# imedslab/OAProgressionMMF

Hardware: AMD Instinct MI355X
Metric: knees/sec full XR+MRI+clin fusion train step (higher is better)
Workload: dtype f32; 1 GPU; syn3: XR1MR3C1CnnTrf train step (fwd+FocalLoss+bwd+Adam), per-GPU batch 8, global batch 8, BASELINE config 4 on BASELINE's synthetic tensors: XR 1x310x310 + 3 x MRI 1x160x384x384 (slice-major) + 9 clinical; random-init weights; parallelism=dp1, activation_recompute=012,012,01

## Files before the change

oaprogressionmmf_amd/csrc/koaf_bn.hip:

```cpp
#include "koaf_cols.h"

namespace {
template <bool H>
__global__ void __launch_bounds__(256) colstats_kernel(const float* __restrict__ x, int64_t rows, int C,
                                                       ColGeom g, float* __restrict__ part, int sq,
                                                       const float* __restrict__ shift) {
    const int t = threadIdx.x, cvx = t % g.CV, ry = t / g.CV;
    const int c0 = blockIdx.y * g.CW;
    const int64_t rbeg = (int64_t)blockIdx.x * g.rpb;
    const int64_t rend = min(rows, rbeg + (int64_t)g.rpb);
    v4f s[2] = {{0, 0, 0, 0}, {0, 0, 0, 0}};
    v4f k = {0, 0, 0, 0};
    if (shift) k = *(const v4f*)&shift[c0 + 4 * cvx];
    for (int64_t r = rbeg + ry; r < rend; r += g.RP) {
        v4f v = load4<H>(x, r * C + c0 + 4 * cvx) - k;
        s[0] += v;
        s[1] += v * v;
    }
    if (sq) col_block_reduce<2>(s, part, blockIdx.x, C, c0, g.CV, g.RP);
    else {
        v4f s1[1] = {s[0]};
        col_block_reduce<1>(s1, part, blockIdx.x, C, c0, g.CV, g.RP);
    }
}

__global__ void colsum_small_kernel(const float* __restrict__ x, int rows, int C, float* __restrict__ out) {
    int c = blockIdx.x * blockDim.x + threadIdx.x;
    if (c >= C) return;
    float a = 0.f;
    for (int r = 0; r < rows; ++r) a += x[(int64_t)r * C + c];
    out[c] = a;
}
}

extern "C" int koaf_colstats(const float* x, int64_t rows, int32_t C, float* part, int32_t* part_rows,
                             const float* shift, int32_t act16, void* stream) {
    ColGeom g;
    KOAF_REQUIRE(x && part && part_rows && rows > 0, "koaf_colstats: bad args");
    KOAF_REQUIRE(col_geom(rows, C, 1024, &g), "koaf_colstats: unsupported C=%d", C);
    KOAF_LAUNCH_ACT16(act16, colstats_kernel<A16>, dim3(g.nblk, g.nchunk), dim3(256), 0, STREAM, x, rows, C, g, part, 1, shift);
    *part_rows = g.nblk;
    return koaf_check_launch("koaf_colstats");
}
extern "C" int32_t koaf_colpart_rows(int64_t rows, int32_t C) {
    ColGeom g;
    if (!col_geom(rows, C, 1024, &g)) return -1;
    return g.nblk;
}

extern "C" int koaf_colsum(const float* x, float* out, int32_t rows, int32_t C, float* part, void* stream) {
    KOAF_REQUIRE(x && out && rows > 0 && C > 0, "koaf_colsum: bad args");
    ColGeom g;
    if (part && aligned16(x) && col_geom(rows, C, 256, &g)) {
        hipLaunchKernelGGL(colstats_kernel<false>, dim3(g.nblk, g.nchunk), dim3(256), 0, STREAM, x, (int64_t)rows, C, g, part,
                           0, (const float*)nullptr);
        hipLaunchKernelGGL(colfinal_kernel<1>, dim3((C + 63) / 64), dim3(1024), 0, STREAM, part, g.nblk, C, out,
                           (float*)nullptr);
    } else {
        hipLaunchKernelGGL(colsum_small_kernel, dim3((C + 255) / 256), dim3(256), 0, STREAM, x, rows, C, out);
    }
    return koaf_check_launch("koaf_colsum");
}
extern "C" int64_t koaf_colsum_ws(int32_t rows, int32_t C) {
    ColGeom g;
    if (!col_geom(rows, C, 256, &g)) return 0;
    return (int64_t)g.nblk * C;
}

namespace {
__global__ void __launch_bounds__(1024) part_reduce_kernel(const float* __restrict__ src, int rows, int C, int nsum,
                                                           int i1, int chunk, double* __restrict__ ws) {
    __shared__ double red[2][16][64];
    const int cx = threadIdx.x & 63, gy = threadIdx.x >> 6;
    const int c = blockIdx.x * 64 + cx;
    const int r0 = blockIdx.y * chunk, r1 = min(rows, r0 + chunk);
    double a = 0.0, b = 0.0;
    if (c < C)
        for (int r = r0 + gy; r < r1; r += 16) {
            a += (double)src[((int64_t)r * nsum + 0) * C + c];
            b += (double)src[((int64_t)r * nsum + i1) * C + c];
        }
    red[0][gy][cx] = a;
// ... 95 lines not shown
    else
        hipLaunchKernelGGL(bn_finalize_kernel<float>, dim3((C + 63) / 64), dim3(1024), 0, STREAM, stats, rows, C, inv,
                           unbias, gamma, beta, running_mean, running_var, num_batches_tracked, momentum, eps, train,
                           mean, invstd, sc, sh, train ? shift : nullptr, koaf_status_ptr());
    return koaf_check_launch("koaf_bn_finalize");
}

namespace {
template <bool H>
__global__ void __launch_bounds__(256) bn_add_relu_kernel(const float* __restrict__ c, const float* __restrict__ sc,
                                                          const float* __restrict__ sh, const float* __restrict__ idt,
                                                          const float* __restrict__ idsc,
                                                          const float* __restrict__ idsh, float* __restrict__ y,
                                                          int64_t nvec, int C4, uint32_t* status) {
    unsigned nsat = 0;
    for (int64_t i = (int64_t)blockIdx.x * EB + threadIdx.x; i < nvec; i += (int64_t)gridDim.x * EB) {
        const int cv = (int)(i % C4) * 4;
        v4f v = load4_nt<H>(c, i * 4);
        const v4f s4 = *(const v4f*)&sc[cv], h4 = *(const v4f*)&sh[cv];
#pragma unroll
        for (int j = 0; j < 4; ++j) v[j] = fmaf(v[j], s4[j], h4[j]);
        if (idt) {
            v4f d = load4_nt<H>(idt, i * 4);
            if (idsc) {
                const v4f is4 = *(const v4f*)&idsc[cv], ih4 = *(const v4f*)&idsh[cv];
#pragma unroll
                for (int j = 0; j < 4; ++j) d[j] = fmaf(d[j], is4[j], ih4[j]);
            }
            v += d;
        }
#pragma unroll
        for (int j = 0; j < 4; ++j) {
            nsat += !(v[j] * KOAF_ACT_SCALE <= 65504.f) ? 1u : 0u;
            v[j] = v[j] != v[j] ? v[j] : fmaxf(v[j], 0.f);
        }
        store4_nt<H>(y, i * 4, v);
    }
    koaf_status_add(status, 0, nsat);
}
}

extern "C" int koaf_bn_add_relu(const float* c, const float* sc, const float* sh, const float* idt, const float* idsc,
                                const float* idsh, float* y, int64_t rows, int32_t C, int32_t act16, void* stream) {
    KOAF_REQUIRE(c && sc && sh && y && rows > 0 && C > 0 && C % 4 == 0, "koaf_bn_add_relu: bad args");
    KOAF_REQUIRE(aligned16(c) && aligned16(y) && aligned16(sc) && aligned16(sh) && (!idt || aligned16(idt)), "koaf_bn_add_relu: unaligned");
    KOAF_REQUIRE((idsc == nullptr) == (idsh == nullptr), "koaf_bn_add_relu: idsc/idsh come together");
    const int64_t nvec = rows * (C / 4);
    KOAF_LAUNCH_ACT16(act16, bn_add_relu_kernel<A16>, dim3(ew_grid(nvec)), dim3(EB), 0, STREAM, c, sc, sh, idt, idsc, idsh, y,
                      nvec, C / 4, koaf_status_ptr());
    return koaf_check_launch("koaf_bn_add_relu");
}
extern "C" int koaf_bn_relu(const float* c, const float* sc, const float* sh, float* y, int64_t rows, int32_t C,
                            int32_t act16, void* stream) {
    return koaf_bn_add_relu(c, sc, sh, nullptr, nullptr, nullptr, y, rows, C, act16, stream);
}

namespace {
struct PoolGeom { const float* g; const uint8_t* am; int H, W, OH, OW; };
template <bool H, bool POOL>
__global__ void __launch_bounds__(256) bn_bwd_reduce_kernel(const float* __restrict__ g, const float* __restrict__ c,
                                                            const float* __restrict__ ymask,
                                                            const float* __restrict__ sc, const float* __restrict__ sh,
                                                            const float* __restrict__ mean,
                                                            const float* __restrict__ invstd, int mask_mode,
                                                            float* __restrict__ dz_out, int64_t rows, int C,
                                                            ColGeom geo, float* __restrict__ part, float* dz_amax, PoolGeom pg) {
    const int t = threadIdx.x, cvx = t % geo.CV, ry = t / geo.CV;
    unsigned am = 0u;
    const int c0 = blockIdx.y * geo.CW + 4 * cvx;
    const int64_t rbeg = (int64_t)blockIdx.x * geo.rpb;
    const int64_t rend = min(rows, rbeg + (int64_t)geo.rpb);
    const v4f mu = *(const v4f*)&mean[c0], is = *(const v4f*)&invstd[c0];
    v4f s4 = {0, 0, 0, 0}, h4 = {0, 0, 0, 0};
    if (mask_mode == 2) { s4 = *(const v4f*)&sc[c0]; h4 = *(const v4f*)&sh[c0]; }
    v4f s[2] = {{0, 0, 0, 0}, {0, 0, 0, 0}};
    int ix = 0, iy = 0, n = 0;
    if constexpr (POOL) {
        int64_t pp = rbeg + ry;
        ix = (int)(pp % pg.W);
        pp /= pg.W;
        iy = (int)(pp % pg.H);
        n = (int)(pp / pg.H);
    }
    for (int64_t r = rbeg + ry; r < rend; r += geo.RP) {
        const int64_t o = r * C + c0;
        v4f gv;
        if constexpr (POOL) {
            gv = (v4f){0.f, 0.f, 0.f, 0.f};
            const int oya = iy >> 1, oyb = (iy + 1) >> 1, oxa = ix >> 1, oxb = (ix + 1) >> 1;
            const bool vy[2] = {oya < pg.OH, oyb != oya && oyb < pg.OH}, vx[2] = {oxa < pg.OW, oxb != oxa && oxb < pg.OW};
            const int oys[2] = {oya, oyb}, oxs[2] = {oxa, oxb};
            uint32_t a4[4];
            v4f gg[4];
#pragma unroll
            for (int wy = 0; wy < 2; ++wy)
#pragma unroll
                for (int wx = 0; wx < 2; ++wx) {
                    const bool ok = vy[wy] && vx[wx];
                    const int64_t po = ok ? ((int64_t)(n * pg.OH + oys[wy]) * pg.OW + oxs[wx]) * C + c0 : (int64_t)c0;
                    a4[2 * wy + wx] = *(const uint32_t*)&pg.am[po];
                    gg[2 * wy + wx] = *(const v4f*)&pg.g[po];
                }
#pragma unroll
            for (int wy = 0; wy < 2; ++wy)
#pragma unroll
                for (int wx = 0; wx < 2; ++wx) {
                    const bool ok = vy[wy] && vx[wx];
                    const uint32_t want = (uint32_t)((iy - (oys[wy] * 2 - 1)) * 3 + (ix - (oxs[wx] * 2 - 1)));
#pragma unroll
                    for (int j = 0; j < 4; ++j)
                        if (ok && ((a4[2 * wy + wx] >> (8 * j)) & 0xffu) == want) gv[j] += gg[2 * wy + wx][j];
                }
            ix += geo.RP;
            while (ix >= pg.W) { ix -= pg.W; if (++iy == pg.H) { iy = 0; ++n; } }
        } else {
            gv = *(const v4f*)&g[o];
        }
        v4f cvv = load4<H>(c, o);
        if (mask_mode == 1) {
            v4f yv = load4<H>(ymask, o);
#pragma unroll
            for (int j = 0; j < 4; ++j) gv[j] = yv[j] > 0.f ? gv[j] : 0.f;
        } else if (mask_mode == 2) {
#pragma unroll
            for (int j = 0; j < 4; ++j) gv[j] = (cvv[j] * s4[j] + h4[j]) > 0.f ? gv[j] : 0.f;
        }
        if (dz_out) *(v4f*)&dz_out[o] = gv;
        s[0] += gv;
        s[1] += gv * ((cvv - mu) * is);
#pragma unroll
        for (int j = 0; j < 4; ++j) am = max(am, koaf_absbits(gv[j]));
    }
    col_block_reduce<2>(s, part, blockIdx.x, C, blockIdx.y * geo.CW, geo.CV, geo.RP);
    if (dz_amax) block_amax_raise_bits(am, dz_amax);
}
}

extern "C" int koaf_bn_bwd_reduce(const float* g, const float* c, const float* ymask, const float* sc, const float* sh,
                                  const float* mean, const float* invstd, int32_t mask_mode, float* dz_out, float* part,
                                  int32_t* part_rows, int64_t rows, int32_t C, float* dz_amax, int32_t act16, void* stream) {
    ColGeom geo;
    KOAF_REQUIRE(g && c && mean && invstd && part && part_rows && rows > 0, "koaf_bn_bwd_reduce: bad args");
    KOAF_REQUIRE(mask_mode != 1 || ymask, "koaf_bn_bwd_reduce: mask_mode 1 needs ymask");
    KOAF_REQUIRE(mask_mode != 2 || (sc && sh), "koaf_bn_bwd_reduce: mask_mode 2 needs sc/sh");
    KOAF_REQUIRE(col_geom(rows, C, 1024, &geo), "koaf_bn_bwd_reduce: unsupported C=%d", C);
    if (dz_amax && hipMemsetAsync(dz_amax, 0, sizeof(float), STREAM) != hipSuccess) {
        koaf_set_error("koaf_bn_bwd_reduce: memset failed");
        return KOAF_ELAUNCH;
    }
    const PoolGeom nopool{nullptr, nullptr, 0, 0, 0, 0};
    KOAF_LAUNCH_ACT16(act16, (bn_bwd_reduce_kernel<A16, false>), dim3(geo.nblk, geo.nchunk), dim3(256), 0, STREAM, g, c, ymask,
                      sc, sh, mean, invstd, mask_mode, dz_out, rows, C, geo, part, dz_amax, nopool);
    *part_rows = geo.nblk;
    return koaf_check_launch("koaf_bn_bwd_reduce");
}

extern "C" int koaf_bn_bwd_reduce_pool(const float* pool_g, const uint8_t* pool_argmax, const float* c, const float* sc,
                                       const float* sh, const float* mean, const float* invstd, float* dz_out, float* part,
                                       int32_t* part_rows, int32_t N, int32_t H, int32_t W, int32_t C, float* dz_amax,
                                       int32_t act16, void* stream) {
    ColGeom geo;
    KOAF_REQUIRE(pool_g && pool_argmax && c && sc && sh && mean && invstd && dz_out && part && part_rows && N > 0 && H > 0 && W > 0,
                 "koaf_bn_bwd_reduce_pool: bad args");
    const int64_t rows = (int64_t)N * H * W;
    KOAF_REQUIRE(col_geom(rows, C, 1024, &geo), "koaf_bn_bwd_reduce_pool: unsupported C=%d", C);
    if (dz_amax && hipMemsetAsync(dz_amax, 0, sizeof(float), STREAM) != hipSuccess) {
        koaf_set_error("koaf_bn_bwd_reduce_pool: memset failed");
        return KOAF_ELAUNCH;
    }
    const PoolGeom pg{pool_g, pool_argmax, H, W, (H + 2 - 3) / 2 + 1, (W + 2 - 3) / 2 + 1};
    KOAF_LAUNCH_ACT16(act16, (bn_bwd_reduce_kernel<A16, true>), dim3(geo.nblk, geo.nchunk), dim3(256), 0, STREAM, nullptr, c,
                      nullptr, sc, sh, mean, invstd, 2, dz_out, rows, C, geo, part, dz_amax, pg);
    *part_rows = geo.nblk;
    return koaf_check_launch("koaf_bn_bwd_reduce_pool");
}

namespace {
template <typename T>
__global__ void __launch_bounds__(1024) bn_bwd_finalize_kernel(const T* __restrict__ part, int rows, int C,
                                                               double inv_count, const float* __restrict__ sc,
                                                               const float* __restrict__ invstd, float* dgamma,
                                                               float* dbeta, float* coef, int nsum, int i1,
                                                               const float* __restrict__ mean,
                                                               const float* __restrict__ dz_amax, double sqrt_nm1,
                                                               float* amax) {
    __shared__ double red[2][16][64];
    float bound = 0.f;
    const int cx = threadIdx.x & 63, gy = threadIdx.x >> 6;
    const int c = blockIdx.x * 64 + cx;
    double a = 0.0, b = 0.0;
    if (c < C)
        for (int r = gy; r < rows; r += 16) {
            a += (double)part[((int64_t)r * nsum + 0) * C + c];
            b += (double)part[((int64_t)r * nsum + i1) * C + c];
        }
    red[0][gy][cx] = a;
    red[1][gy][cx] = b;
    __syncthreads();
    if (gy == 0 && c < C) {
        double s1 = 0.0, s2 = 0.0;
        for (int j = 0; j < 16; ++j) { s1 += red[0][j][cx]; s2 += red[1][j][cx]; }
        if (dbeta) dbeta[c] = (float)s1;
        if (dgamma) dgamma[c] = (float)s2;
        const float k0 = sc[c], k1 = (float)(s1 * inv_count), k2 = (float)((double)sc[c] * (double)invstd[c] * s2 * inv_count);
        coef[c] = k0;
        coef[C + c] = k1;
        coef[2 * C + c] = k2;
        if (mean) {
            coef[3 * C + c] = k2 * mean[c] - k0 * k1;
            if (amax) bound = fabsf(k0) * ((dz_amax ? *dz_amax : 0.f) + fabsf(k1)) + fabsf(k2) * (float)(sqrt_nm1 / (double)invstd[c]);
        }
    }
    if (amax && mean) block_amax_raise(bound, amax);
}
// ... 243 lines not shown
```

oaprogressionmmf_amd/csrc/koaf_conv.hip:

```cpp
#include "koaf_common.h"

namespace {

inline int64_t rup32(int64_t v) { return (v + 31) / 32 * 32; }

inline void set_fimg(KoafGemm* g, const KoafWImg* w, int R, int64_t K) {
    g->fmt = 1;
    g->A.fscale = KOAF_ACT_SCALE;
    g->B.amax = w->amax;
    if (!w->f) return;
    g->B.kind = 2; g->B.gather = 0;
    g->B.planes = w->f; g->B.ld = rup32(K); g->B.plane_stride = (int64_t)R * g->B.ld;
}

inline void set_aplanes(KoafOperand* a, const uint16_t* planes, int64_t plane_elems) {
    a->kind = 2; a->planes = planes; a->plane_stride = plane_elems; a->zeros = planes + 2 * plane_elems;
    a->ptr = nullptr; a->ptr2 = nullptr; a->tf = 0; a->sc = a->sh = a->sc2 = nullptr;
}

inline void set_gather(KoafOperand* o, int gather, int H, int W, int C, int CS, int PH, int PW, int KH, int KW, int stride, int pad_h,
                       int pad_w) {
    o->gather = gather;
    o->H = H; o->W = W; o->C = C; o->CS = CS;
    o->PH = PH; o->PW = PW;
// ... 188 lines not shown
                g.B.C = Cout; g.B.ld = (int64_t)KH * KW * Cin;
                g.B.KW = g.A.KW; g.B.tap_stride = 2ll * Cin; g.B.tap_stride_h = 2ll * KW * Cin;
                if (ps) {
                    g.B.kind = 2; g.B.gather = 0;
                    g.B.planes = w_dimg + ((int64_t)khs * KW + kws) * Cout; g.B.ld = dld; g.B.plane_stride = dps;
                    g.B.tap_stride = 2ll * Cout; g.B.tap_stride_h = 2ll * KW * Cout;
                }
                if (dy_planes && nkh > 0 && nkw > 0) set_aplanes(&g.A, dy_planes, (int64_t)N * OH * OW * Cout);
                g.M = N * Hc * Wc; g.N = Cin; g.K = nkh * nkw * Cout;
                g.C = dx; g.ldc = Cin;
                g.residual = residual; g.ldr = Cin;
                g.cmap = 1; g.cm_PH = Hc; g.cm_PW = Wc; g.cm_H = H; g.cm_W = W; g.cm_py = py; g.cm_px = px;
                if (bnb) {
                    set_bnb(&g, bnb, part + (int64_t)rows_done * nsum * Cin);
                    rows_done += koaf_gemm_part_rows(&g);
                }
                g.act16 = act16 ? 2 : 0;
                int rc = koaf_gemm(&g, stream);
                if (rc != KOAF_OK) return rc;
            }
        if (part_rows) *part_rows = rows_done;
        return KOAF_OK;
    }
    zero_gemm(&g);
    g.prec = 1;
    if (f16) { g.fmt = 1; g.A.amax = dy_amax; g.B.amax = wimg->amax; }
    g.A.ptr = dy;
    g.A.kind = 0;
    if (dy_apply) set_apply(&g.A, dy_apply, Cout);
    g.B.ptr = w;
    g.B.kind = 1;
    if (is_pointwise(KH, KW, stride, pad)) {
        g.A.gather = 0;
        g.A.ld = Cout;
        g.B.gather = 0;
        g.B.ld = Cin;
    } else {
        set_gather(&g.A, 2, OH, OW, Cout, Cout, H, W, KH, KW, stride, pad, pad);
        g.B.gather = 3;
        g.B.C = Cout;
        g.B.ld = (int64_t)KH * KW * Cin;
        g.B.KW = KW;
        g.B.tap_stride = Cin;
        g.B.tap_stride_h = (int64_t)KW * Cin;
    }
    if (ps) {
        g.B.kind = 2; g.B.gather = 0; g.B.C = 0; g.B.tap_stride = g.B.tap_stride_h = 0;
        g.B.planes = w_dimg; g.B.ld = dld; g.B.plane_stride = dps;
    }
    if (dy_planes) set_aplanes(&g.A, dy_planes, (int64_t)N * OH * OW * Cout);
    g.M = (int)M; g.N = Cin; g.K = KH * KW * Cout;
    g.C = dx; g.ldc = Cin;
    g.residual = residual; g.ldr = Cin;
    if (bnb) {
        set_bnb(&g, bnb, part);
        *part_rows = koaf_gemm_part_rows(&g);
    }
    g.act16 = act16 ? 2 : 0;
    return koaf_gemm(&g, stream);
}

extern "C" int koaf_conv2d_dgrad(const float* dy, const float* w, float* dx, int32_t N, int32_t H, int32_t W,
                                 int32_t Cin, int32_t Cout, int32_t KH, int32_t KW, int32_t stride, int32_t pad,
                                 const float* residual, const KoafWImg* wimg, const float* dy_amax,
                                 const KoafBnApply* dy_apply, const uint16_t* dy_planes, int32_t act16, void* stream) {
    return koaf_conv2d_dgrad_bnb(dy, w, dx, N, H, W, Cin, Cout, KH, KW, stride, pad, residual, nullptr, nullptr,
                                 nullptr, wimg, dy_amax, dy_apply, dy_planes, act16, stream);
}

bool koaf_wgrad3_ring_ok(int N, int H, int W, int Cin, int Cout);
int64_t koaf_wgrad3_ring_ws(int N, int H, int W, int Cin, int Cout);
int koaf_wgrad3_ring(const uint16_t* dy_planes, const uint16_t* x_planes, float* dw, float* slabs, const float* dy_amax,
                     float x_scale, int N, int H, int W, int Cin, int Cout, void* stream);
static inline bool wgrad3_ring_shape(int N, int H, int W, int Cin, int Cout, int KH, int KW, int stride, int pad) {
    return KH == 3 && KW == 3 && stride == 1 && pad == 1 && koaf_wgrad3_ring_ok(N, H, W, Cin, Cout);
}

int koaf_wgrad1(const KoafGemm& g, int bm, int bn, void* stream);
constexpr int WGRAD1_MIN_KCHUNK = 1024;
static inline WgradPlan wgrad1_tile(const KoafGemm& g, const WgradPlan& p) {
    WgradPlan t = {0, 0, p.splitk};
    const KoafOperand& B = g.B;
    if (g.fmt != 1 || g.act16 != 0 || g.A.kind != 1 || B.kind != 1 || g.A.gather || (B.gather != 0 && B.gather != 1)) return t;
    if (g.M % 128 || g.N % 128 || (g.M < 256 && g.N < 256)) return t;
    const int bm = g.M >= 256 ? 256 : 128, bn = g.N >= 256 ? 256 : 128;
    if (g.M % bm || g.N % bn) return t;
    if (B.gather == 1) {
        const bool f11 = B.KH == 1 && B.KW == 1 && B.pad == 0 && B.pad_w == 0, f33 = B.KH == 3 && B.KW == 3 && B.pad == 1 && B.pad_w == 1;
        if (B.stride != 2 || !(f11 || f33) || B.CS != B.C || B.C % bn || B.PH <= 0 || B.PW <= 0) return t;
        if ((int64_t)(g.K / (B.PH * B.PW)) * B.H * B.W >= (1ll << 31)) return t;
    }
    if (rup32(cdiv64(g.K, p.splitk)) < WGRAD1_MIN_KCHUNK) return t;
    if (!aligned16(g.A.ptr) || !aligned16(g.B.ptr) || !aligned16(g.C)) return t;
    if (g.A.tf && (!aligned16(g.A.ptr2) || !aligned16(g.A.sc) || !aligned16(g.A.sh) || !aligned16(g.A.sc2))) return t;
    if (g.B.tf && (!aligned16(g.B.sc) || !aligned16(g.B.sh))) return t;
    t.bm = bm; t.bn = bn;
    return t;
}

extern "C" int64_t koaf_conv2d_wgrad_ws(int32_t N, int32_t H, int32_t W, int32_t Cin, int32_t Cout, int32_t KH,
                                        int32_t KW, int32_t stride, int32_t pad) {
    const int OH = conv_out(H, KH, stride, pad), OW = conv_out(W, KW, stride, pad);
    WgradPlan p = wgrad_plan(Cout, KH * KW * Cin, (int64_t)N * OH * OW, Cin, 1);
    int64_t ws = p.splitk > 1 ? (int64_t)(p.splitk + 16) * Cout * KH * KW * Cin : 0;
    if (wgrad3_ring_shape(N, H, W, Cin, Cout, KH, KW, stride, pad)) {
        const int64_t w3 = koaf_wgrad3_ring_ws(N, H, W, Cin, Cout);
        if (w3 > ws) ws = w3;
    }
    return ws;
}

extern "C" int koaf_conv2d_wgrad(const float* dy, const float* x, float* dw, int32_t N, int32_t H, int32_t W,
                                 int32_t Cin, int32_t Cout, int32_t KH, int32_t KW, int32_t stride, int32_t pad,
                                 const float* in_sc, const float* in_sh, float* slabs, const float* dy_amax,
                                 const KoafBnApply* dy_apply, const uint16_t* dy_planes, const uint16_t* x_planes,
                                 int32_t act16, void* stream) {
    KOAF_REQUIRE((dy_planes == nullptr) == (x_planes == nullptr) && (!dy_planes || dy_amax || dy_apply),
                 "koaf_conv2d_wgrad: dy_planes and x_planes come together, with dy_amax (or dy_apply)");
    KOAF_REQUIRE((dy || dy_apply || dy_planes) && (x || x_planes) && dw && N > 0 && Cin % 64 == 0 && Cout % 4 == 0, "koaf_conv2d_wgrad: bad args");
    KOAF_REQUIRE(!dy_apply || (dy_apply->dz && dy_apply->c && dy_apply->coef && dy_apply->amax),
                 "koaf_conv2d_wgrad: dy_apply needs dz / c / coef / amax");
    if (dy_apply) { dy = dy_apply->dz; dy_amax = dy_apply->amax; }
    KOAF_REQUIRE((in_sc == nullptr) == (in_sh == nullptr), "koaf_conv2d_wgrad: in_sc/in_sh come together");
    const int OH = conv_out(H, KH, stride, pad), OW = conv_out(W, KW, stride, pad);
    const int64_t P = (int64_t)N * OH * OW;
    KOAF_REQUIRE(P < (1ll << 31), "koaf_conv2d_wgrad: too many pixels");
    const int Ntot = KH * KW * Cin;
    if (dy_planes && slabs && wgrad3_ring_shape(N, H, W, Cin, Cout, KH, KW, stride, pad))
        return koaf_wgrad3_ring(dy_planes, x_planes, dw, slabs, dy_amax, KOAF_ACT_SCALE, N, H, W, Cin, Cout, stream);
    WgradPlan p = wgrad_plan(Cout, Ntot, P, Cin, 1);
    KOAF_REQUIRE(p.splitk == 1 || slabs, "koaf_conv2d_wgrad: workspace required");
    KoafGemm g;
    zero_gemm(&g);
    g.prec = 1;
    if (dy_amax) { g.fmt = 1; g.A.amax = dy_amax; g.B.fscale = KOAF_ACT_SCALE; }
    g.A.ptr = dy; g.A.kind = 1; g.A.ld = Cout;
    if (dy_apply) set_apply(&g.A, dy_apply, Cout);
    g.B.ptr = x; g.B.kind = 1;
    if (is_pointwise(KH, KW, stride, pad)) {
        g.B.gather = 0;
        g.B.ld = Cin;
    } else
        set_gather(&g.B, 1, H, W, Cin, Cin, OH, OW, KH, KW, stride, pad, pad);
    if (in_sc) { g.B.tf = 1; g.B.sc = in_sc; g.B.sh = in_sh; }
    if (dy_planes) {
        set_aplanes(&g.A, dy_planes, P * Cout);
        g.A.kind = 3; g.A.ld = Cout;
        set_aplanes(&g.B, x_planes, (int64_t)N * H * W * Cin);
        g.B.kind = 3;
        set_gather(&g.B, 1, H, W, Cin, Cin, OH, OW, KH, KW, stride, pad, pad);
    }
    g.M = Cout; g.N = Ntot; g.K = (int)P;
    g.bm = p.bm; g.bn = p.bn; g.splitk = p.splitk;
    g.C = p.splitk > 1 ? slabs : dw;
    g.ldc = Ntot;
    g.act16 = (act16 && !dy_planes) ? 3 : 0;
    const WgradPlan t1 = wgrad1_tile(g, p);
    int rc = t1.bm ? koaf_wgrad1(g, t1.bm, t1.bn, stream) : koaf_gemm(&g, stream);
    if (rc != KOAF_OK || p.splitk == 1) return rc;
    return koaf_slab_reduce(slabs, p.splitk, (int64_t)Cout * Ntot, dw, stream);
}

extern "C" int koaf_gconv_expand_w(const float* w, float* wexp, int32_t C, int32_t groups, float* amax, void* stream) {
    KOAF_REQUIRE(w && wexp && C % 64 == 0 && groups > 0 && C % groups == 0 && 64 % (C / groups) == 0,
                 "koaf_gconv_expand_w: C=%d groups=%d unsupported", C, groups);
    hipLaunchKernelGGL(gconv_expand_kernel, dim3(1024), dim3(256), 0, STREAM, w, wexp, C, C / groups, amax);
    return koaf_check_launch("koaf_gconv_expand_w");
}
// ... 94 lines not shown
```

oaprogressionmmf_amd/csrc/koaf_wgrad1.hip:

```cpp
#include <hip/hip_runtime.h>
#include <stdint.h>
#include <type_traits>
#include "koaf.h"
#include "koaf_pieces.h"

namespace {
struct Wg1Params {
    const float* a;
    const float* a2;
    const float* asc;
    const float* ash;
    const float* asc2;
    const float* a_amax;
    const float* b;
    const float* bsc;
    const float* bsh;
    float b_scale;
    float* out;
    uint32_t* status;
    int M, N, K, splitk;
    int H, W, C, PH, PW, KW, stride, pad, pad_w;
};

constexpr int WG1_NT = 512;

constexpr int WG1_TAB = 4 * BK;
constexpr unsigned WG1_INVALID = 0x80000000u;

template <int R, int TF, bool G = false>
struct Wg1Loader {
    static constexpr int NU = R / 64;
    static constexpr int CV = R / 4;
    static constexpr int RP = WG1_NT / CV;
    static constexpr int SK = R / 2 + 16;
    static constexpr int PL = plane_dwords(R, false);
    v4f r[NU];
    v4f r2[TF == 2 ? NU : 1];
    v4f ca, cb, ck;
    const float* src;
    const float* src2;
    float fsc;
    unsigned ld, col, kr;
    unsigned vm;

    __device__ __forceinline__ void init(const float* p, const float* p2, const float* sc, const float* sh, const float* sc2,
                                         int c0, int ldim, float scale) {
        const unsigned t = threadIdx.x;
        src = p; src2 = p2;
        fsc = scale;
        ld = (unsigned)ldim;
        col = (unsigned)c0 + 4u * (t % CV);
        kr = t / CV;
        vm = 0u;
        ca = cb = ck = (v4f){0.f, 0.f, 0.f, 0.f};
        if constexpr (TF != 0) {
            ca = *(const v4f*)(sc + col) * fsc;
            cb = *(const v4f*)(sh + col) * fsc;
            if constexpr (TF == 2) ck = *(const v4f*)(sc2 + col) * fsc;
        }
    }
    __device__ __forceinline__ void issue(int i, int k0, int K) {
        const int kb = min(k0, K - 1);
        const unsigned rowmax = (unsigned)(K - 1 - kb);
        const unsigned row = min(kr + (unsigned)(RP * i), rowmax);
        const unsigned off = __umul24(row, ld) + col;
        const int64_t base = (int64_t)kb * ld;
        r[i] = *(const v4f*)(src + base + off);
        if constexpr (TF == 2) r2[i] = *(const v4f*)(src2 + base + off);
    }
    __device__ __forceinline__ void issue_g(int i, const unsigned* T) {
        const unsigned e = T[kr + (unsigned)(RP * i)];
        vm = (vm & ~(1u << i)) | ((e >> 31) << i);
        const uint64_t off = (uint64_t)(e & ~WG1_INVALID) * ld + col;
        r[i] = *(const v4f*)(src + off);
    }
    template <bool FULL>
    __device__ __forceinline__ void convert(int i, int klim, unsigned* S) {
        constexpr float HMAX = 65504.f;
        const bool ok = G ? ((vm >> i) & 1u) == 0u : (FULL || (int)(kr + (unsigned)(RP * i)) < klim);
        v4f v;
#pragma unroll
        for (int j = 0; j < 4; ++j) {
            float x = r[i][j];
            if constexpr (TF == 1) {
                x = fmaf(x, ca[j], cb[j]);
                x = __builtin_amdgcn_fmed3f(x, 0.f, HMAX);
            } else if constexpr (TF == 2) {
                x = fmaf(ca[j], x, fmaf(-ck[j], r2[i][j], cb[j]));
                x = __builtin_amdgcn_fmed3f(x, -HMAX, HMAX);
            } else {
                x = __builtin_amdgcn_fmed3f(x * fsc, -HMAX, HMAX);
            }
            v[j] = ok ? x : 0.f;
        }
        unsigned pl[2][2];
        split2h(v, pl);
        const unsigned off = (kr + (unsigned)(RP * i)) * SK + 2u * (threadIdx.x % CV);
#pragma unroll
        for (int q = 0; q < 2; ++q) *(uint2*)&S[q * PL + off] = make_uint2(pl[q][0], pl[q][1]);
    }
};

template <int BM, int BN, int TFA, int TFB, bool GB>
__global__ void __launch_bounds__(WG1_NT) wgrad1_kernel(const Wg1Params p) {
    constexpr int WGM = 4, WGN = 2;
    constexpr int WM = BM / WGM, WN = BN / WGN, TM = WM / 32, TN = WN / 32;
    typedef Wg1Loader<BM, TFA> LA;
    typedef Wg1Loader<BN, TFB, GB> LB;
    constexpr int A_ELEMS = 2 * LA::PL, B_ELEMS = 2 * LB::PL, STAGE = A_ELEMS + B_ELEMS;
    static_assert((2 * STAGE + WG1_TAB) * 4 <= 160 * 1024, "two stages of both operands in LDS");
    __shared__ __attribute__((aligned(16))) unsigned smem[2 * STAGE + (GB ? WG1_TAB : 0)];
    [[maybe_unused]] unsigned* const tab = smem + 2 * STAGE;

    const int ntn = p.N / BN;
    unsigned bid = blockIdx.x;
    int split = blockIdx.y;
    if (gridDim.y > 1 && (gridDim.y & 7) == 0) {
        const unsigned lin = blockIdx.x + gridDim.x * blockIdx.y, x = lin & 7, slot = lin >> 3;
        bid = slot % gridDim.x;
        split = (int)((slot / gridDim.x) * 8 + x);
    }
    const int tn = bid % ntn, tm = bid / ntn;
    const int m0 = tm * BM, n0 = tn * BN;
    const int kchunk = (((p.K + p.splitk - 1) / p.splitk + BK - 1) / BK) * BK;
    const int kbeg = split * kchunk;
    const int kend = min(p.K, kbeg + kchunk);
    const int klen = max(kend - kbeg, 0), nstep = (klen + BK - 1) / BK;

    const float sca = scale_of_amax(*p.a_amax), scb = p.b_scale;
    float alpha = 1.f / (sca * scb);
    if (!koaf_bits_finite(koaf_absbits(*p.a_amax))) {
        alpha = __uint_as_float(0x7fc00000u);
        if (blockIdx.x == 0 && blockIdx.y == 0 && threadIdx.x == 0) koaf_status_add(p.status, 1, 1u);
    }

    LA la;
    LB lb;
    la.init(p.a, p.a2, p.asc, p.ash, p.asc2, m0, p.M, sca);
    [[maybe_unused]] int g_kh = 0, g_kw = 0;
    if constexpr (GB) {
        const int tap = n0 / p.C;
        g_kh = tap / p.KW;
        g_kw = tap - g_kh * p.KW;
        lb.init(p.b, nullptr, p.bsc, p.bsh, nullptr, n0 - tap * p.C, p.C, scb);
    } else
        lb.init(p.b, nullptr, p.bsc, p.bsh, nullptr, n0, p.N, scb);
    [[maybe_unused]] auto table = [&](int j, int lane32) {
        const int k = kbeg + j * BK + lane32;
        const unsigned kk = (unsigned)min(k, p.K - 1), ppi = (unsigned)(p.PH * p.PW);
        const unsigned n = kk / ppi, rem = kk - n * ppi, oy = rem / (unsigned)p.PW, ox = rem - oy * (unsigned)p.PW;
        const int sy = (int)oy * p.stride - p.pad + g_kh, sx = (int)ox * p.stride - p.pad_w + g_kw;
        const bool ok = k < kend && (unsigned)sy < (unsigned)p.H && (unsigned)sx < (unsigned)p.W;
        tab[(j & 3) * BK + lane32] = ok ? (n * (unsigned)p.H + (unsigned)sy) * (unsigned)p.W + (unsigned)sx : WG1_INVALID;
    };

    const int t = threadIdx.x, lane = t & 63, w = t >> 6;
    const int wm = w / WGN, wn = w % WGN;

    v16f acc[TM][TN];
#pragma unroll
    for (int i = 0; i < TM; ++i)
#pragma unroll
        for (int j = 0; j < TN; ++j)
#pragma unroll
            for (int e = 0; e < 16; ++e) acc[i][j][e] = 0.f;

    constexpr int NUT = LA::NU + LB::NU, NG = 2 * TN;
    auto unit = [&](auto full, int u, int klim, unsigned* S, int k2) {
        constexpr bool FULL = decltype(full)::value;
        if (u < LA::NU) {
            la.template convert<FULL>(u, klim, S);
            la.issue(u, k2, p.K);
        } else {
            lb.template convert<FULL>(u - LA::NU, klim, S + A_ELEMS);
            if constexpr (GB) lb.issue_g(u - LA::NU, tab + (((k2 - kbeg) / BK) & 3) * BK);
            else lb.issue(u - LA::NU, k2, p.K);
        }
    };
    auto step = [&](auto full, int cur, int klim, int k2) {
        const unsigned* Au = smem + cur * STAGE;
        const unsigned* Bu = Au + A_ELEMS;
        unsigned* Sn = smem + (cur ^ 1) * STAGE;
        if constexpr (GB) {
            if (threadIdx.x < BK) table((k2 - kbeg) / BK + 1, threadIdx.x);
        }
#pragma unroll
        for (int g = 0; g < 2; ++g) {
            v4i ap[TM][2];
#pragma unroll
            for (int i = 0; i < TM; ++i)
#pragma unroll
                for (int q = 0; q < 2; ++q) ap[i][q] = frag_load<BM, false>(Au + q * LA::PL, wm * WM + 32 * i, g, lane);
#pragma unroll
            for (int jn = 0; jn < TN; ++jn) {
                v4i bp[2];
#pragma unroll
                for (int q = 0; q < 2; ++q) bp[q] = frag_load<BN, false>(Bu + q * LB::PL, wn * WN + 32 * jn, g, lane);
                constexpr int PAH[3] = {1, 0, 0}, PBH[3] = {0, 1, 0};
#pragma unroll
                for (int term = 0; term < 3; ++term)
#pragma unroll
                    for (int i = 0; i < TM; ++i)
                        acc[i][jn] = __builtin_amdgcn_mfma_f32_32x32x16_f16(__builtin_bit_cast(h16x8, ap[i][PAH[term]]),
                                                                            __builtin_bit_cast(h16x8, bp[PBH[term]]), acc[i][jn], 0, 0, 0);
                const int grp = g * TN + jn;
#pragma unroll
                for (int u = 0; u < NUT; ++u)
                    if (u * NG / NUT == grp) unit(full, u, klim, Sn, k2);
                __builtin_amdgcn_sched_barrier(0x104);
            }
        }
        asm volatile("s_waitcnt lgkmcnt(0)\n\ts_barrier" ::: "memory");
    };

    if (nstep > 0) {
        if constexpr (GB) {
            if (threadIdx.x < 3 * BK) table(threadIdx.x / BK, threadIdx.x % BK);
            asm volatile("s_waitcnt lgkmcnt(0)\n\ts_barrier" ::: "memory");
        }
#pragma unroll
        for (int i = 0; i < LA::NU; ++i) la.issue(i, kbeg, p.K);
#pragma unroll
        for (int i = 0; i < LB::NU; ++i) {
            if constexpr (GB) lb.issue_g(i, tab);
            else lb.issue(i, kbeg, p.K);
        }
#pragma unroll
        for (int u = 0; u < NUT; ++u) unit(std::false_type{}, u, klen, smem, kbeg + BK);
        asm volatile("s_waitcnt lgkmcnt(0)\n\ts_barrier" ::: "memory");
    }
    const int nfull = max(klen / BK - 1, 0);
    int s = 0;
#pragma unroll 1
    for (; s < nfull; ++s) step(std::true_type{}, s & 1, BK, kbeg + (s + 2) * BK);
#pragma unroll 1
    for (; s < nstep; ++s) step(std::false_type{}, s & 1, klen - (s + 1) * BK, kbeg + (s + 2) * BK);

    float* out = p.out + (p.splitk > 1 ? (int64_t)split * p.M * p.N : (int64_t)0);
    const int r = lane & 31, h = lane >> 5;
#pragma unroll
    for (int i = 0; i < TM; ++i)
#pragma unroll
        for (int jn = 0; jn < TN; ++jn)
#pragma unroll
            for (int e = 0; e < 16; ++e) {
                float v = alpha * acc[i][jn][e];
                asm volatile("" : "+v"(v));
                v += 0.f;
                const int row = m0 + wm * WM + 32 * i + (e & 3) + 8 * (e >> 2) + 4 * h;
                const int col = n0 + wn * WN + 32 * jn + r;
                out[(int64_t)row * p.N + col] = v;
            }
}

template <int BM, int BN, bool GB>
int wg1_launch(const Wg1Params& p, int tfa, int tfb, dim3 grid, hipStream_t s) {
#define WG1_GO(TA, TB) hipLaunchKernelGGL((wgrad1_kernel<BM, BN, TA, TB, GB>), grid, dim3(WG1_NT), 0, s, p)
    if (tfa == 2) { if (tfb) WG1_GO(2, 1); else WG1_GO(2, 0); }
    else { if (tfb) WG1_GO(0, 1); else WG1_GO(0, 0); }
#undef WG1_GO
    return koaf_check_launch("koaf_wgrad1");
}
template <bool GB>
int wg1_tile(const Wg1Params& p, int bm, int bn, int tfa, int tfb, dim3 grid, hipStream_t s) {
    if (bm == 256 && bn == 256) return wg1_launch<256, 256, GB>(p, tfa, tfb, grid, s);
    if (bm == 256) return wg1_launch<256, 128, GB>(p, tfa, tfb, grid, s);
    return wg1_launch<128, 256, GB>(p, tfa, tfb, grid, s);
}
}

void koaf_log_launch(const char* variant, const KoafGemm& g, dim3 grid, dim3 launched);

int koaf_wgrad1(const KoafGemm& g, int bm, int bn, void* stream) {
    const KoafOperand& B = g.B;
    const bool gb = B.gather == 1;
    KOAF_REQUIRE(g.fmt == 1 && g.act16 == 0 && g.A.kind == 1 && B.kind == 1 && !g.A.gather && (B.gather == 0 || gb) && g.A.amax && g.A.ptr && B.ptr &&
                 g.C && (g.A.tf == 0 || (g.A.tf == 2 && g.A.ptr2 && g.A.sc && g.A.sh && g.A.sc2)) && (B.tf == 0 || (B.tf == 1 && B.sc && B.sh)) &&
                 (bm == 256 || bm == 128) && (bn == 256 || bn == 128) && bm + bn >= 384 && g.M % bm == 0 && g.N % bn == 0 && g.K >= BK && g.K < (1 << 30) &&
                 g.splitk >= 1 && g.splitk <= 65535 && g.A.ld == g.M && (gb || B.ld == g.N) && g.ldc == g.N,
                 "koaf_wgrad1: bad args");
    KOAF_REQUIRE(!gb || (B.stride == 2 && B.KH == B.KW && B.pad == B.pad_w && ((B.KH == 1 && B.pad == 0) || (B.KH == 3 && B.pad == 1)) &&
                         (B.CS == 0 || B.CS == B.C) && B.C % bn == 0 && g.N == B.KH * B.KW * B.C && B.PH > 0 && B.PW > 0 &&
                         B.PH == (B.H + 2 * B.pad - B.KH) / 2 + 1 && B.PW == (B.W + 2 * B.pad_w - B.KW) / 2 + 1 && g.K % (B.PH * B.PW) == 0 &&
                         (int64_t)(g.K / (B.PH * B.PW)) * B.H * B.W < (1ll << 31)),
                 "koaf_wgrad1: bad gather");
    Wg1Params p;
    p.a = g.A.ptr; p.a2 = g.A.ptr2; p.asc = g.A.sc; p.ash = g.A.sh; p.asc2 = g.A.sc2; p.a_amax = g.A.amax;
    p.b = B.ptr; p.bsc = B.sc; p.bsh = B.sh;
    p.b_scale = B.fscale != 0.f ? B.fscale : 1.f;
    p.out = g.C;
    p.status = g.status ? g.status : koaf_status_ptr();
    p.M = g.M; p.N = g.N; p.K = g.K; p.splitk = g.splitk;
    p.H = B.H; p.W = B.W; p.C = B.C; p.PH = B.PH; p.PW = B.PW; p.KW = B.KW; p.stride = B.stride; p.pad = B.pad; p.pad_w = B.pad_w;
    const dim3 grid((unsigned)((g.M / bm) * (g.N / bn)), (unsigned)g.splitk);
    KoafGemm rec = g;
    rec.bm = bm; rec.bn = bn;
    koaf_log_launch("koaf_wgrad1", rec, grid, grid);
    hipStream_t s = (hipStream_t)stream;
    return gb ? wg1_tile<true>(p, bm, bn, g.A.tf, B.tf, grid, s) : wg1_tile<false>(p, bm, bn, g.A.tf, B.tf, grid, s);
}
```

Measured before the change: 4.194 knees/s.

## Add narrow 64-wide wgrad1 tiles and nontemporal unrolled BN backward reduce

Lets the split-K 1x1 weight-gradient kernel take 64-wide M or N shapes (64x64, 64x256, 256x64) with a smaller wave grid, leaving surplus waves idle. These shapes previously went to a slower fallback path. Separately, the non-pooled BN backward reduce loop is unrolled by two rows and uses nontemporal loads and stores to cut cache pollution on streaming data. The narrow tiles leave some waves with no work, and nontemporal hints could hurt if the data is reused soon after.

```diff
diff --git a/oaprogressionmmf_amd/csrc/koaf_bn.hip b/oaprogressionmmf_amd/csrc/koaf_bn.hip
--- a/oaprogressionmmf_amd/csrc/koaf_bn.hip
+++ b/oaprogressionmmf_amd/csrc/koaf_bn.hip
@@ -1,3 +1,4 @@
+#include <type_traits>
 #include "koaf_cols.h"
 
 namespace {
@@ -259,11 +260,44 @@
         iy = (int)(pp % pg.H);
         n = (int)(pp / pg.H);
     }
-    for (int64_t r = rbeg + ry; r < rend; r += geo.RP) {
-        const int64_t o = r * C + c0;
-        v4f gv;
-        if constexpr (POOL) {
-            gv = (v4f){0.f, 0.f, 0.f, 0.f};
+    auto row = [&](v4f gv, const v4f cvv, const v4f yv, const int64_t o, auto nt) {
+        if (mask_mode == 1) {
+#pragma unroll
+            for (int j = 0; j < 4; ++j) gv[j] = yv[j] > 0.f ? gv[j] : 0.f;
+        } else if (mask_mode == 2) {
+#pragma unroll
+            for (int j = 0; j < 4; ++j) gv[j] = (cvv[j] * s4[j] + h4[j]) > 0.f ? gv[j] : 0.f;
+        }
+        if (dz_out) {
+            if constexpr (decltype(nt)::value) __builtin_nontemporal_store(gv, (v4f*)&dz_out[o]);
+            else *(v4f*)&dz_out[o] = gv;
+        }
+        s[0] += gv;
+        s[1] += gv * ((cvv - mu) * is);
+#pragma unroll
+        for (int j = 0; j < 4; ++j) am = max(am, koaf_absbits(gv[j]));
+    };
+    if constexpr (!POOL) {
+        const v4f zero = {0.f, 0.f, 0.f, 0.f};
+        const int64_t step = (int64_t)geo.RP * C;
+        int64_t r = rbeg + ry;
+        for (; r + geo.RP < rend; r += 2 * geo.RP) {
+            const int64_t o0 = r * C + c0, o1 = o0 + step;
+            const v4f g0 = __builtin_nontemporal_load((const v4f*)&g[o0]), g1 = __builtin_nontemporal_load((const v4f*)&g[o1]);
+            const v4f c0v = load4_nt<H>(c, o0), c1v = load4_nt<H>(c, o1);
+            v4f y0 = zero, y1 = zero;
+            if (mask_mode == 1) { y0 = load4_nt<H>(ymask, o0); y1 = load4_nt<H>(ymask, o1); }
+            row(g0, c0v, y0, o0, std::true_type{});
+            row(g1, c1v, y1, o1, std::true_type{});
+        }
+        if (r < rend) {
+            const int64_t o = r * C + c0;
+            row(__builtin_nontemporal_load((const v4f*)&g[o]), load4_nt<H>(c, o), mask_mode == 1 ? load4_nt<H>(ymask, o) : zero, o, std::true_type{});
+        }
+    } else {
+        for (int64_t r = rbeg + ry; r < rend; r += geo.RP) {
+            const int64_t o = r * C + c0;
+            v4f gv = {0.f, 0.f, 0.f, 0.f};
             const int oya = iy >> 1, oyb = (iy + 1) >> 1, oxa = ix >> 1, oxb = (ix + 1) >> 1;
             const bool vy[2] = {oya < pg.OH, oyb != oya && oyb < pg.OH}, vx[2] = {oxa < pg.OW, oxb != oxa && oxb < pg.OW};
             const int oys[2] = {oya, oyb}, oxs[2] = {oxa, oxb};
@@ -290,23 +324,8 @@
                 }
             ix += geo.RP;
             while (ix >= pg.W) { ix -= pg.W; if (++iy == pg.H) { iy = 0; ++n; } }
-        } else {
-            gv = *(const v4f*)&g[o];
-        }
-        v4f cvv = load4<H>(c, o);
-        if (mask_mode == 1) {
-            v4f yv = load4<H>(ymask, o);
-#pragma unroll
-            for (int j = 0; j < 4; ++j) gv[j] = yv[j] > 0.f ? gv[j] : 0.f;
-        } else if (mask_mode == 2) {
-#pragma unroll
-            for (int j = 0; j < 4; ++j) gv[j] = (cvv[j] * s4[j] + h4[j]) > 0.f ? gv[j] : 0.f;
-        }
-        if (dz_out) *(v4f*)&dz_out[o] = gv;
-        s[0] += gv;
-        s[1] += gv * ((cvv - mu) * is);
-#pragma unroll
-        for (int j = 0; j < 4; ++j) am = max(am, koaf_absbits(gv[j]));
+            row(gv, load4<H>(c, o), (v4f){0.f, 0.f, 0.f, 0.f}, o, std::false_type{});
+        }
     }
     col_block_reduce<2>(s, part, blockIdx.x, C, blockIdx.y * geo.CW, geo.CV, geo.RP);
     if (dz_amax) block_amax_raise_bits(am, dz_amax);
diff --git a/oaprogressionmmf_amd/csrc/koaf_conv.hip b/oaprogressionmmf_amd/csrc/koaf_conv.hip
--- a/oaprogressionmmf_amd/csrc/koaf_conv.hip
+++ b/oaprogressionmmf_amd/csrc/koaf_conv.hip
@@ -294,8 +294,9 @@
     WgradPlan t = {0, 0, p.splitk};
     const KoafOperand& B = g.B;
     if (g.fmt != 1 || g.act16 != 0 || g.A.kind != 1 || B.kind != 1 || g.A.gather || (B.gather != 0 && B.gather != 1)) return t;
-    if (g.M % 128 || g.N % 128 || (g.M < 256 && g.N < 256)) return t;
-    const int bm = g.M >= 256 ? 256 : 128, bn = g.N >= 256 ? 256 : 128;
+    const bool narrow = B.gather == 0 && (g.M == 64 || g.M == 256) && (g.N == 64 || g.N == 256) && (g.M == 64 || g.N == 64);
+    if (!narrow && (g.M % 128 || g.N % 128 || (g.M < 256 && g.N < 256))) return t;
+    const int bm = narrow ? g.M : g.M >= 256 ? 256 : 128, bn = narrow ? g.N : g.N >= 256 ? 256 : 128;
     if (g.M % bm || g.N % bn) return t;
     if (B.gather == 1) {
         const bool f11 = B.KH == 1 && B.KW == 1 && B.pad == 0 && B.pad_w == 0, f33 = B.KH == 3 && B.KW == 3 && B.pad == 1 && B.pad_w == 1;
diff --git a/oaprogressionmmf_amd/csrc/koaf_wgrad1.hip b/oaprogressionmmf_amd/csrc/koaf_wgrad1.hip
--- a/oaprogressionmmf_amd/csrc/koaf_wgrad1.hip
+++ b/oaprogressionmmf_amd/csrc/koaf_wgrad1.hip
@@ -103,8 +103,10 @@
 
 template <int BM, int BN, int TFA, int TFB, bool GB>
 __global__ void __launch_bounds__(WG1_NT) wgrad1_kernel(const Wg1Params p) {
-    constexpr int WGM = 4, WGN = 2;
+    constexpr int WGM = BM >= 128 ? 4 : 2, WGN = 8 / WGM < BN / 32 ? 8 / WGM : BN / 32;
+    constexpr bool ALLW = WGM * WGN == WG1_NT / 64;
     constexpr int WM = BM / WGM, WN = BN / WGN, TM = WM / 32, TN = WN / 32;
+    static_assert(TM >= 1 && TN >= 1 && WM % 32 == 0 && WN % 32 == 0, "a wave tile is whole 32 x 32 accumulators");
     typedef Wg1Loader<BM, TFA> LA;
     typedef Wg1Loader<BN, TFB, GB> LB;
     constexpr int A_ELEMS = 2 * LA::PL, B_ELEMS = 2 * LB::PL, STAGE = A_ELEMS + B_ELEMS;
@@ -156,6 +158,7 @@
 
     const int t = threadIdx.x, lane = t & 63, w = t >> 6;
     const int wm = w / WGN, wn = w % WGN;
+    [[maybe_unused]] const bool mw = ALLW || w < WGM * WGN;
 
     v16f acc[TM][TN];
 #pragma unroll
@@ -187,22 +190,26 @@
 #pragma unroll
         for (int g = 0; g < 2; ++g) {
             v4i ap[TM][2];
-#pragma unroll
-            for (int i = 0; i < TM; ++i)
-#pragma unroll
-                for (int q = 0; q < 2; ++q) ap[i][q] = frag_load<BM, false>(Au + q * LA::PL, wm * WM + 32 * i, g, lane);
+            if (mw) {
+#pragma unroll
+                for (int i = 0; i < TM; ++i)
+#pragma unroll
+                    for (int q = 0; q < 2; ++q) ap[i][q] = frag_load<BM, false>(Au + q * LA::PL, wm * WM + 32 * i, g, lane);
+            }
 #pragma unroll
             for (int jn = 0; jn < TN; ++jn) {
-                v4i bp[2];
-#pragma unroll
-                for (int q = 0; q < 2; ++q) bp[q] = frag_load<BN, false>(Bu + q * LB::PL, wn * WN + 32 * jn, g, lane);
-                constexpr int PAH[3] = {1, 0, 0}, PBH[3] = {0, 1, 0};
-#pragma unroll
-                for (int term = 0; term < 3; ++term)
-#pragma unroll
-                    for (int i = 0; i < TM; ++i)
-                        acc[i][jn] = __builtin_amdgcn_mfma_f32_32x32x16_f16(__builtin_bit_cast(h16x8, ap[i][PAH[term]]),
-                                                                            __builtin_bit_cast(h16x8, bp[PBH[term]]), acc[i][jn], 0, 0, 0);
+                if (mw) {
+                    v4i bp[2];
+#pragma unroll
+                    for (int q = 0; q < 2; ++q) bp[q] = frag_load<BN, false>(Bu + q * LB::PL, wn * WN + 32 * jn, g, lane);
+                    constexpr int PAH[3] = {1, 0, 0}, PBH[3] = {0, 1, 0};
+#pragma unroll
+                    for (int term = 0; term < 3; ++term)
+#pragma unroll
+                        for (int i = 0; i < TM; ++i)
+                            acc[i][jn] = __builtin_amdgcn_mfma_f32_32x32x16_f16(__builtin_bit_cast(h16x8, ap[i][PAH[term]]),
+                                                                                __builtin_bit_cast(h16x8, bp[PBH[term]]), acc[i][jn], 0, 0, 0);
+                }
                 const int grp = g * TN + jn;
 #pragma unroll
                 for (int u = 0; u < NUT; ++u)
@@ -238,6 +245,7 @@
 
     float* out = p.out + (p.splitk > 1 ? (int64_t)split * p.M * p.N : (int64_t)0);
     const int r = lane & 31, h = lane >> 5;
+    if (!mw) return;
 #pragma unroll
     for (int i = 0; i < TM; ++i)
 #pragma unroll
@@ -263,6 +271,11 @@
 }
 template <bool GB>
 int wg1_tile(const Wg1Params& p, int bm, int bn, int tfa, int tfb, dim3 grid, hipStream_t s) {
+    if constexpr (!GB) {
+        if (bm == 256 && bn == 64) return wg1_launch<256, 64, false>(p, tfa, tfb, grid, s);
+        if (bm == 64 && bn == 256) return wg1_launch<64, 256, false>(p, tfa, tfb, grid, s);
+        if (bm == 64) return wg1_launch<64, 64, false>(p, tfa, tfb, grid, s);
+    }
     if (bm == 256 && bn == 256) return wg1_launch<256, 256, GB>(p, tfa, tfb, grid, s);
     if (bm == 256) return wg1_launch<256, 128, GB>(p, tfa, tfb, grid, s);
     return wg1_launch<128, 256, GB>(p, tfa, tfb, grid, s);
@@ -276,7 +289,8 @@
     const bool gb = B.gather == 1;
     KOAF_REQUIRE(g.fmt == 1 && g.act16 == 0 && g.A.kind == 1 && B.kind == 1 && !g.A.gather && (B.gather == 0 || gb) && g.A.amax && g.A.ptr && B.ptr &&
                  g.C && (g.A.tf == 0 || (g.A.tf == 2 && g.A.ptr2 && g.A.sc && g.A.sh && g.A.sc2)) && (B.tf == 0 || (B.tf == 1 && B.sc && B.sh)) &&
-                 (bm == 256 || bm == 128) && (bn == 256 || bn == 128) && bm + bn >= 384 && g.M % bm == 0 && g.N % bn == 0 && g.K >= BK && g.K < (1 << 30) &&
+                 (((bm == 256 || bm == 128) && (bn == 256 || bn == 128) && bm + bn >= 384) ||
+                  (!gb && (bm == 256 || bm == 64) && (bn == 256 || bn == 64) && (bm == 64 || bn == 64))) && g.M % bm == 0 && g.N % bn == 0 && g.K >= BK && g.K < (1 << 30) &&
                  g.splitk >= 1 && g.splitk <= 65535 && g.A.ld == g.M && (gb || B.ld == g.N) && g.ldc == g.N,
                  "koaf_wgrad1: bad args");
     KOAF_REQUIRE(!gb || (B.stride == 2 && B.KH == B.KW && B.pad == B.pad_w && ((B.KH == 1 && B.pad == 0) || (B.KH == 3 && B.pad == 1)) &&
```

Result: no change. 4.210 knees/s (median of 6 runs) (+0.4%).
